# AllenNeuralDynamics/aind-exaspim-image-compression

Measured on AMD Instinct MI355X. Metric: denoised+encoded voxels/s on 1024^3 uint16, higher is better.
Workload: dtype f32

## Files before the change

aind-exaspim-image-compression_amd/csrc/bm_kernels.hip:

```cpp
#include "exabm4d_kernels.h"
#ifdef EXABM4D_BM_STAMPS
#define KERNEL_STAMPS
#endif
#include "kernel_stamps.h"
#include <type_traits>
#include <utility>

namespace exabm4d {

#ifdef EXABM4D_BM_STAMPS
__device__ unsigned long long g_bm_stamps[8];
__device__ unsigned long long g_bm_barrier_stamps[4][8];
#endif

struct __attribute__((packed, aligned(4))) float4u {
    float x, y, z, w;
};
template <class F, int... I>
__device__ __forceinline__ void static_for(F&& f, std::integer_sequence<int, I...>) {
    (f(std::integral_constant<int, I>{}), ...);
}

constexpr int TCZ = 8;
constexpr int NE = 6;
constexpr int NSTEP = SWIN * 2 * 4;
template <int TCY_, int TCX_>
struct TilePlan {
    static constexpr int TCY = TCY_, TCX = TCX_;
    static constexpr int TRY = TCY - 1, TRX = TCX - 1;
    static constexpr int PROWS = 4 * (TCY - 1) + 3 + NE;
    static_assert(TCY * TCX == 64, "one wave per cell layer");
};
template <int TCY_, int TCX_>
struct TileShape : TilePlan<TCY_, TCX_> {
    using Plan = TilePlan<TCY_, TCX_>;
    static constexpr int PCOLS = 4 * (TCX_ - 1) + 16;
    static constexpr int PSTR = TCX_ == 8 ? 56 : PCOLS;
    static constexpr int PCH = PSTR / 4;
    static constexpr int NDMA = (Plan::PROWS * PCH + 63) / 64;
    static constexpr int PLANE = (Plan::PROWS * PSTR + 3) / 4 * 4;
    static constexpr int PBUF = PLANE > 2144 ? PLANE : 2144;
    static_assert(PCOLS % 4 == 0 && PSTR % 4 == 0, "whole 16-byte chunks");
};

constexpr int CARRY_ROUND = (NE / 2) * SWIN * 64;
constexpr int CARRY_TILE = (NSTEP / 4) * 2 * CARRY_ROUND;
struct Carry {
    int on;
    int strip;
    uint32_t* buf;
    int* done;
    int* ticket;
    unsigned* status;
    int fault;
};
constexpr int CARRY_POLL_LIMIT = 1 << 23;
template <class T, class D>
__device__ __forceinline__ void carry_prefetch(const T* src, D* dst, int lane) {
    static_assert(2 * CARRY_ROUND == 16 * 256 + 128, "two rounds = 16.5 KB");
#pragma unroll
    for (int i = 0; i < 16; i++)
        __builtin_amdgcn_global_load_lds((const __attribute__((address_space(1))) void*)(src + 256 * i + 4 * lane),
                                         (__attribute__((address_space(3))) void*)(dst + 256 * i), 16, 0, 17);
    if (lane < 32)
        __builtin_amdgcn_global_load_lds((const __attribute__((address_space(1))) void*)(src + 4096 + 4 * lane),
                                         (__attribute__((address_space(3))) void*)(dst + 4096), 16, 0, 17);
}
__device__ __forceinline__ void carry_wait_for(const int* done, int tiles, int lane, const Carry& carry) {
    if (lane == 0) {
        int polls = carry.fault ? CARRY_POLL_LIMIT : 0;
        while (__hip_atomic_load(done, __ATOMIC_RELAXED, __HIP_MEMORY_SCOPE_SYSTEM) < tiles) {
            if (++polls > CARRY_POLL_LIMIT) {
                __hip_atomic_fetch_or(carry.status, 1u, __ATOMIC_RELAXED, __HIP_MEMORY_SCOPE_SYSTEM);
                break;
            }
            __builtin_amdgcn_s_sleep(32);
        }
        if (carry.fault) __hip_atomic_fetch_or(carry.status, 1u, __ATOMIC_RELAXED, __HIP_MEMORY_SCOPE_SYSTEM);
    }
}
__device__ __forceinline__ int launch_position(const Carry& carry, int quota) {
    if (!carry.on) return (int)blockIdx.x;
    __shared__ int s_pos;
    if (threadIdx.x == 0) {
        const int xcc = (int)(__builtin_amdgcn_s_getreg((4 - 1) << 11 | 0 << 6 | 20) & 7);
        int pos = -1;
        for (int k = 0; k < 8 && pos < 0; k++) {
            const int c = (xcc + k) & 7;
            const int j = __hip_atomic_fetch_add(carry.ticket + c, 1, __ATOMIC_RELAXED, __HIP_MEMORY_SCOPE_AGENT);
            if (j < quota) pos = 8 * j + c;
        }
        s_pos = pos;
    }
    __syncthreads();
    return s_pos;
}

struct TileId {
    int tz, col, cols;
    int bi, ty, tx;
};
__device__ __forceinline__ bool tile_id(TileId& t, int tiles_y, int tiles_x, int xcd_q, int nbatch,
                                        const Carry& carry) {
    const int per = tiles_y * tiles_x;
    t.cols = per * nbatch;
    if (xcd_q) {
        const int lp = launch_position(carry, (int)(gridDim.x >> 3));
        const int s = lp < 0 ? -1 : xcd_slab_sync(lp, t.cols, xcd_q);
        if (s < 0) return false;
        t.tz = s / t.cols;
        t.col = s - t.tz * t.cols;
    } else {
// ... 245 lines not shown
                            const uint32_t cbase =
                                1u + (uint32_t)(((dz + RAD) * SWIN + (dy + RAD)) * SWIN);
                            const bool self_row = (dz == 0) && (dy == 0);
#pragma unroll
                            for (int d = 0; d < SWIN; d++) {
                                const float* c0 = lo_w + (cz == 0 && e0 ? CARRY_ROUND : 0) + 64 * ((e - e0) * SWIN + d);
                                const float* c1 = up_w + 64 * ((e - e0) * SWIN + d);
                                float s0 = c0[0] + c0[TCX];
                                asm("" : "+v"(s0));
                                const float s1 = c1[0] + c1[TCX];
                                const float S = s0 + s1;
                                const uint32_t code = (d == RAD && self_row) ? 0u : cbase + d;
                                const bool valid = vzy && ((xmask >> d) & 1u);
                                list_admit(list, thr, keymax, __float_as_uint(S), code, valid);
                            }
                        }
                    }
                }
                __syncthreads();
                if (carries) {
#pragma unroll
                    for (int e = e0; e < e0 + NE / 2; e++)
#pragma unroll
                        for (int d = 0; d < SWIN; d++) {
                            const float right = __int_as_float(__builtin_amdgcn_update_dpp(
                                0, __float_as_int(acc[e][d]), 0x101 , 0xF, 0xF, true));
                            __hip_atomic_store(cslot + (e0 ? CARRY_ROUND : 0) + 64 * ((e - e0) * SWIN + d), acc[e][d] + right,
                                               __ATOMIC_RELAXED, __HIP_MEMORY_SCOPE_SYSTEM);
                        }
                }
            }
#pragma unroll
            for (int e = 0; e < NE; e++)
#pragma unroll
                for (int d = 0; d < SWIN; d++) acc[e][d] = 0.0f;
        }

        if (!xin && step + 1 < NSTEP) stage_edge(step + 1, nxt);
    }

    if (ref_ok) list_store(keys + ((size_t)((size_t)iz * g.gy + iy) * g.gx + ix) * MAXG, list);
    } while (false);

    if (carry.on) {
        asm volatile("s_waitcnt vmcnt(0)" ::: "memory");
        __syncthreads();
        if (threadIdx.x == 0) __hip_atomic_store(done_col, tz + 1, __ATOMIC_RELAXED, __HIP_MEMORY_SCOPE_SYSTEM);
    }
}

typedef short s16x2 __attribute__((ext_vector_type(2)));
typedef uint32_t u32x2 __attribute__((ext_vector_type(2)));
typedef uint32_t u32x4 __attribute__((ext_vector_type(4)));
template <int TCY_, int TCX_>
struct TileShape16 : TilePlan<TCY_, TCX_> {
    using Plan = TilePlan<TCY_, TCX_>;
    static constexpr int PCOLS = ((4 * TCX_ + 10 + 7) / 8) * 8;
    static constexpr int PSTR = TCX_ == 8 ? 56 : 80;
    static constexpr int PCH = PSTR / 8;
    static constexpr int NDMA = (Plan::PROWS * PCH + 63) / 64;
    static constexpr int PLANE_DW = NDMA * 256;
    static constexpr int XCH_DW = (NE / 2) * SWIN * 64;
    static constexpr int PBUF = PLANE_DW > XCH_DW ? PLANE_DW : XCH_DW;
    static_assert(PCOLS <= PSTR, "staged columns fit the row");
};

template <class TS>
__global__ __launch_bounds__(512) void bm_tile16_kernel(const uint16_t* __restrict__ vol_all, VolGeom g,
                                                        uint32_t keymax,
                                                        uint32_t* __restrict__ keys_all, int tiles_y,
                                                        int tiles_x, int xcd_q, int nbatch, Carry carry) {
    constexpr int TCX = TS::TCX, TRX = TS::TRX, TRY = TS::TRY, PROWS = TS::PROWS, PCOLS = TS::PCOLS,
                  PSTR = TS::PSTR, PCH = TS::PCH, NDMA = TS::NDMA, PBUF = TS::PBUF;
    __shared__ __align__(16) uint32_t pbuf_all[TCZ][2][PBUF];
    __shared__ __align__(16) uint32_t lower0[2 * CARRY_ROUND + 64];

    TileId id;
    if (!tile_id(id, tiles_y, tiles_x, xcd_q, nbatch, carry)) return;
    const int tz = id.tz, col = id.col, cols = id.cols, bi = id.bi, ty = id.ty, tx = id.tx;
    const uint16_t* __restrict__ vol = vol_all + (size_t)bi * (size_t)g.nvox;
    uint32_t* __restrict__ keys = keys_all + (size_t)bi * (size_t)g.nref * MAXG;
    const int tid = threadIdx.x;
    const int lane = tid & 63;
    const int cx = lane % TCX, cy = lane / TCX, cz = __builtin_amdgcn_readfirstlane(tid >> 6);
    const int ix = TRX * tx + cx, iy = TRY * ty + cy;
    const size_t sy = (size_t)g.nx, sz = (size_t)g.nx * (size_t)g.ny;
#ifdef EXABM4D_BM_STAMPS
    unsigned long long st[8] = {}, stb[4] = {};
    const unsigned long long tk0 = stamp();
#endif

    const int Ls = (carry.on ? TCZ : TCZ - 1) * tz;
    const uint32_t* carry_rd = carry.buf + ((size_t)((tz + 1) & 1) * cols + col) * CARRY_TILE;
    uint32_t* carry_wr = carry.buf + ((size_t)(tz & 1) * cols + col) * CARRY_TILE;
    int* done_col = carry.done + col;

    const int qy = min(STEP * iy, g.ny - STEP), qx = min(STEP * ix, g.nx - STEP);
    const int Y0 = STEP * TRY * ty, X0 = STEP * TRX * tx - RAD - 1;
    const int ry = STEP * iy, rx = STEP * ix;
    const bool ref_yx = cx < TRX && cy < TRY && iy < g.ay && ix < g.ax;

    uint32_t xmask = 0;
#pragma unroll
    for (int d = 0; d < SWIN; d++)
        xmask |= ((rx + d - RAD >= 0) && (rx + d - RAD <= g.nx - BLK)) ? (1u << d) : 0u;

    do {
    const int L = Ls + cz;
    const bool active = L <= g.az;
    const int iz = L - 1;
    const int qz = min(STEP * L, g.nz - STEP);
    const int Z0 = STEP * L;
    const bool lower_carried = carry.on && cz == 0 && tz > 0;
    const bool carries = carry.on && cz == TCZ - 1 && L + 1 <= g.az;
    const bool ref_ok = ref_yx && active && (cz > 0 || lower_carried);
    {
        STAMP(c0);
        if ((lower_carried || carries) && tz > 0) carry_wait_for(done_col, tz, lane, carry);
        STAMP(c1);
        STAMP_ADD(6, c0, c1);
    }
    const int rz = STEP * iz;

    uint32_t list[MAXG];
#pragma unroll
    for (int k = 0; k < MAXG; k++) list[k] = KEY_EMPTY;
    uint32_t thr = keymax;

    uint32_t doff[2][NDMA], coff[4];
    int yb[2];
    {
        int l = lane;
        asm volatile("" : "+v"(l));
#pragma unroll
        for (int ps = 0; ps < 2; ps++) {
            const int dylo = ps == 0 ? -RAD : 1;
            yb[ps] = min(max(Y0 + dylo, 0), g.ny - 1);
#pragma unroll
            for (int i = 0; i < NDMA; i++) {
                const unsigned p = 64u * i + (unsigned)l;
                const unsigned r0 = (p * (65536u / PCH + 1u)) >> 16;
                const unsigned r = min(r0, (unsigned)(PROWS - 1));
                const unsigned q = min(p - r0 * PCH, (unsigned)(PCOLS / 8 - 1));
                const int yy = min(max(Y0 + dylo + (int)r, 0), g.ny - 1);
                doff[ps][i] = 2u * ((unsigned)(yy - yb[ps]) * (unsigned)g.nx + 8u * q);
                asm volatile("" : "+v"(doff[ps][i]));
            }
        }
#pragma unroll
        for (int y = 0; y < 4; y++) {
            coff[y] = 2u * ((unsigned)(qy - Y0 + y) * (unsigned)g.nx + (unsigned)qx);
            asm volatile("" : "+v"(coff[y]));
        }
    }
    const char* const vol_b = reinterpret_cast<const char*>(vol);
    u32x2 An[4];
    auto load_cell_plane = [&](int step) {
        const char* cbase = vol_b + 2 * ((long long)(qz + (step & 3)) * (long long)sz + (long long)Y0 * (long long)sy);
#pragma unroll
        for (int y = 0; y < 4; y++) {
            uint32_t o = coff[y];
            asm volatile("" : "+v"(o));
            const uint32_t* ap = reinterpret_cast<const uint32_t*>(cbase + (size_t)o);
            An[y] = u32x2{ap[0], ap[1]};
        }
    };

    using lds_u32 = __attribute__((address_space(3))) uint32_t;
    auto pbuf = [&](int w, int b) { return (lds_u32*)&pbuf_all[w][b][0]; };
    auto issue_dma = [&](int step, lds_u32* dst) {
        const int z = step & 3, pass = (step >> 2) & 1, dz = (step >> 3) - RAD;
        const int pz = min(max(Z0 + z + dz, 0), g.nz - 1);
        const int yb0 = yb[0], yb1 = yb[1];
        const char* base = vol_b + 2 * ((long long)pz * (long long)sz +
                                        (long long)(pass ? yb1 : yb0) * (long long)sy + X0);
#pragma unroll
        for (int i = 0; i < NDMA; i++) {
            const uint32_t o0 = doff[0][i], o1 = doff[1][i];
            __builtin_amdgcn_global_load_lds(
                (const __attribute__((address_space(1))) void*)(base + (size_t)(pass ? o1 : o0)),
                (__attribute__((address_space(3))) void*)(dst + 256 * i), 16, 0, 0);
        }
    };

    if (!active) {
        for (int i = 0; i < (NSTEP / 4) * 4; i++) __syncthreads();
        break;
    }
    issue_dma(0, pbuf(cz, 0));
    load_cell_plane(0);
    asm volatile("" ::"v"(An[0]), "v"(An[1]), "v"(An[2]), "v"(An[3]));

    int acc[NE][SWIN];
#pragma unroll
    for (int e = 0; e < NE; e++)
#pragma unroll
        for (int d = 0; d < SWIN; d++) acc[e][d] = 0;

    auto step_body = [&](auto NEc, const int step) {
        constexpr int NEP = decltype(NEc)::value;
        const int z = step & 3;
        lds_u32* cur = pbuf(cz, step & 1);
        lds_u32* nxt = pbuf(cz, (step + 1) & 1);

        STAMP(t0);
        asm volatile("s_waitcnt vmcnt(0)" ::: "memory");
        STAMP(t1);
        (void)load_cell_plane;
        const u32x2 A[4] = {An[0], An[1], An[2], An[3]};
        STAMP(t2);
        if (step + 1 < NSTEP) issue_dma(step + 1, nxt);
        if (lower_carried && z == 2)
            carry_prefetch(carry_rd + (size_t)(step >> 2) * 2 * CARRY_ROUND, (lds_u32*)&lower0[0], lane);
        if (step + 1 < NSTEP) load_cell_plane(step + 1);
        asm volatile("" ::: "memory");
        STAMP(t3);

        {
            const lds_u32* wrow_l = cur + ((4 * cy) * PSTR + 4 * cx) / 2;
            const uint32_t wrow_lds = (uint32_t)(uintptr_t)wrow_l;
            auto read_row = [&](auto rc, u32x4& lo, u32x4& hi) {
                constexpr int r = decltype(rc)::value;
                constexpr int O = r * (PSTR / 4);
                static_assert(O + 3 < 256, "ds_read2_b64 offsets are 8 bits");
                const uint32_t row0 = wrow_lds;
                asm volatile("ds_read2_b64 %0, %2 offset0:%3 offset1:%4\n\t"
                             "ds_read2_b64 %1, %2 offset0:%5 offset1:%6"
                             : "=&v"(lo), "=&v"(hi)
                             : "v"(row0), "n"(O), "n"(O + 1), "n"(O + 2), "n"(O + 3));
            };
            auto await_row = [&](u32x4& lo, u32x4& hi) {
                asm volatile("s_waitcnt lgkmcnt(0)" : "+v"(lo), "+v"(hi));
            };
            u32x4 q0, q1;
            read_row(std::integral_constant<int, 0>{}, q0, q1);
            await_row(q0, q1);
            STAMP(t4);
            static_for([&](auto rc) {
                constexpr int rp = decltype(rc)::value;
                u32x4 n0, n1;
                if constexpr (rp + 1 < 3 + NEP) read_row(std::integral_constant<int, rp + 1>{}, n0, n1);
                asm volatile("" ::: "memory");
                const uint32_t W[8] = {q0.x, q0.y, q0.z, q0.w, q1.x, q1.y, q1.z, q1.w};
                uint32_t Wo[7];
#pragma unroll
                for (int i = 0; i < 7; i++) Wo[i] = __builtin_amdgcn_alignbit(W[i + 1], W[i], 16);
#pragma unroll
                for (int y = 0; y < 4; y++) {
                    const int e = rp - y;
                    if (e >= 0 && e < NEP) {
#pragma unroll
                        for (int xp = 0; xp < 2; xp++) {
                            const s16x2 a = __builtin_bit_cast(s16x2, xp ? A[y].y : A[y].x);
#pragma unroll
                            for (int d = 0; d < SWIN; d++) {
                                const int j = 1 + 2 * xp + d;
                                const uint32_t wp = (j & 1) ? Wo[(j - 1) / 2] : W[j / 2];
                                const s16x2 t = __builtin_elementwise_sub_sat(a, __builtin_bit_cast(s16x2, wp));
                                acc[e][d] = __builtin_amdgcn_sdot2(t, t, acc[e][d], true);
                            }
                        }
                    }
                }
                if constexpr (rp + 1 < 3 + NEP) {
                    await_row(n0, n1);
                    q0 = n0;
                    q1 = n1;
                }
            }, std::make_integer_sequence<int, 3 + NEP>{});
            asm volatile("" ::: "memory");
            STAMP(t5);
            STAMP_ADD(0, t0, t1);
            STAMP_ADD(1, t1, t2);
            STAMP_ADD(2, t3, t4);
            STAMP_ADD(3, t4, t5);
        }
    };
    auto pass_end = [&](auto NEc, const int step) {
        constexpr int NEP = decltype(NEc)::value;
        constexpr int NR0 = (NEP + 1) / 2;
        const int dz = (step >> 3) - RAD;
        const int dylo = NEP == NE ? -RAD : 1;
        lds_u32* cur = pbuf(cz, step & 1);
        {
            const bool vz = (rz + dz >= 0) && (rz + dz <= g.nz - BLK);
            lds_u32* mine = cur + lane;
            const lds_u32* up_w = cur + lane;
            const lds_u32* lo_w = (cz > 0 ? pbuf(max(cz - 1, 0), step & 1) : (lds_u32*)&lower0[0]) + lane;
            uint32_t* cslot = carry_wr + (size_t)((step >> 2) * 2) * CARRY_ROUND + lane;
            auto pair_sum = [&](int e, int d) {
                const uint32_t c = min((uint32_t)acc[e][d], 1u << 27);
                const uint32_t right = (uint32_t)__builtin_amdgcn_update_dpp(
                    0, (int)c, 0x101 , 0xF, 0xF, true);
                return c + right;
            };
#pragma unroll
            for (int e0 = 0; e0 < NEP; e0 += NR0) {
#pragma unroll
                for (int e = e0; e < (e0 + NR0 < NEP ? e0 + NR0 : NEP); e++)
#pragma unroll
                    for (int d = 0; d < SWIN; d++) mine[64 * ((e - e0) * SWIN + d)] = pair_sum(e, d);
                STAMP(b0);
                __syncthreads();
                STAMP(b1);
                if (ref_ok) {
#pragma unroll
                    for (int e = e0; e < (e0 + NR0 < NEP ? e0 + NR0 : NEP); e++) {
                        uint32_t Sv[1][SWIN];
#pragma unroll
                        for (int d = 0; d < SWIN; d++) {
                            const lds_u32* c0 = lo_w + (cz == 0 && e0 ? CARRY_ROUND : 0) + 64 * ((e - e0) * SWIN + d);
                            const lds_u32* c1 = up_w + 64 * ((e - e0) * SWIN + d);
                            Sv[0][d] = (c0[0] + c0[TCX]) + (c1[0] + c1[TCX]);
                        }
                        asm volatile("" ::: "memory");
                        const int dy = dylo + e;
                        {
                            const bool vzy = vz && (ry + dy >= 0) && (ry + dy <= g.ny - BLK);
                            const uint32_t cbase =
                                1u + (uint32_t)(((dz + RAD) * SWIN + (dy + RAD)) * SWIN);
                            const bool self_row = (dz == 0) && (dy == 0);
#pragma unroll
                            for (int d = 0; d < SWIN; d++) {
                                const uint32_t S = Sv[0][d];
                                const uint32_t code = (d == RAD && self_row) ? 0u : cbase + d;
                                const bool valid = vzy && ((xmask >> d) & 1u);
                                list_admit(list, thr, keymax, __float_as_uint((float)S), code, valid);
                            }
                        }
                    }
                }
                STAMP(b2);
                __syncthreads();
                STAMP(b3);
                STAMP_ADD(4, b0, b1);
                STAMP_ADD(5, b1, b2);
                STAMP_ADD(4, b2, b3);
#ifdef EXABM4D_BM_STAMPS
                stb[e0 ? 2 : 0] += b1 - b0;
                stb[e0 ? 3 : 1] += b3 - b2;
#endif
                if (carries) {
                    uint32_t* cw = cslot + (size_t)(e0 ? CARRY_ROUND : 0);
#pragma unroll
                    for (int e = e0; e < (e0 + NR0 < NEP ? e0 + NR0 : NEP); e++)
#pragma unroll
                        for (int d = 0; d < SWIN; d++)
                            __hip_atomic_store(cw + 64 * ((e - e0) * SWIN + d), pair_sum(e, d), __ATOMIC_RELAXED,
                                               __HIP_MEMORY_SCOPE_SYSTEM);
                }
            }
#pragma unroll
            for (int e = 0; e < NE; e++)
#pragma unroll
                for (int d = 0; d < SWIN; d++) acc[e][d] = 0;
        }
    };
    static_assert(NSTEP == 8 * SWIN, "two passes of four planes per dz");
#pragma unroll 1
    for (int step0 = 0; step0 < NSTEP; step0 += 8) {
#pragma unroll 1
        for (int step = step0; step < step0 + 4; step++) step_body(std::integral_constant<int, NE>{}, step);
        pass_end(std::integral_constant<int, NE>{}, step0 + 3);
#pragma unroll 1
        for (int step = step0 + 4; step < step0 + 8; step++) step_body(std::integral_constant<int, NE - 1>{}, step);
        pass_end(std::integral_constant<int, NE - 1>{}, step0 + 7);
    }

    if (ref_ok) list_store(keys + ((size_t)((size_t)iz * g.gy + iy) * g.gx + ix) * MAXG, list);
    } while (false);

    if (carry.on) {
        STAMP(c0);
        asm volatile("s_waitcnt vmcnt(0)" ::: "memory");
        __syncthreads();
        STAMP(c1);
        STAMP_ADD(6, c0, c1);
        if (threadIdx.x == 0) __hip_atomic_store(done_col, tz + 1, __ATOMIC_RELAXED, __HIP_MEMORY_SCOPE_SYSTEM);
    }
#ifdef EXABM4D_BM_STAMPS
    st[7] = stamp() - tk0;
    if (lane == 0)
        for (int i = 0; i < 8; i++) atomicAdd(&g_bm_stamps[i], st[i]);
    if (lane == 0)
        for (int i = 0; i < 4; i++) atomicAdd(&g_bm_barrier_stamps[i][tid >> 6], stb[i]);
#endif
}

#ifdef EXABM4D_BM_STAMPS
extern "C" void exabm4d_debug_bm_stamps(unsigned long long* out, int reset) {
    unsigned long long z[8] = {};
    (void)hipDeviceSynchronize();
    (void)hipMemcpyFromSymbol(out, HIP_SYMBOL(g_bm_stamps), sizeof(z));
    if (reset) (void)hipMemcpyToSymbol(HIP_SYMBOL(g_bm_stamps), z, sizeof(z));
}
extern "C" void exabm4d_debug_bm_barrier_stamps(unsigned long long* out, int reset) {
    unsigned long long z[4][8] = {};
    (void)hipDeviceSynchronize();
    (void)hipMemcpyFromSymbol(out, HIP_SYMBOL(g_bm_barrier_stamps), sizeof(z));
    if (reset) (void)hipMemcpyToSymbol(HIP_SYMBOL(g_bm_barrier_stamps), z, sizeof(z));
}
#endif

__global__ __launch_bounds__(64) void bm_generic_kernel(const float* __restrict__ vol_all,
                                                        VolGeom g, uint32_t keymax,
                                                        uint32_t* __restrict__ keys_all,
                                                        int only_unaligned) {
    __shared__ float rb[BVOX];
    const float* __restrict__ vol = vol_all + (size_t)blockIdx.y * (size_t)g.nvox;
    uint32_t* __restrict__ keys = keys_all + (size_t)blockIdx.y * (size_t)g.nref * MAXG;

    const long long r = blockIdx.x;
    const int ix = (int)(r % g.gx), iy = (int)((r / g.gx) % g.gy),
              iz = (int)(r / ((long long)g.gx * g.gy));
    if (only_unaligned && iz < g.az && iy < g.ay && ix < g.ax) return;
    const int rz = grid_pos(iz, g.az, g.nz), ry = grid_pos(iy, g.ay, g.ny),
              rx = grid_pos(ix, g.ax, g.nx);
    const size_t sy = (size_t)g.nx, sz = (size_t)g.nx * (size_t)g.ny;
    const int lane = threadIdx.x;

    for (int i = lane; i < BVOX; i += 64) {
        const int bx = i & 7, by = (i >> 3) & 7, bz = i >> 6;
        rb[i] = vol[(size_t)(rz + bz) * sz + (size_t)(ry + by) * sy + (rx + bx)];
    }
    __syncthreads();

    uint32_t list[MAXG];
#pragma unroll
    for (int k = 0; k < MAXG; k++) list[k] = KEY_EMPTY;

    for (int c = lane; c < NCAND; c += 64) {
        const int dx = c % SWIN - RAD, dy = (c / SWIN) % SWIN - RAD, dz = c / (SWIN * SWIN) - RAD;
        const int pz = rz + dz, py = ry + dy, px = rx + dx;
        const bool valid = pz >= 0 && pz <= g.nz - BLK && py >= 0 && py <= g.ny - BLK && px >= 0 &&
                           px <= g.nx - BLK;
        uint32_t key = KEY_EMPTY;
        if (valid) {
            const float* __restrict__ b = vol + (size_t)pz * sz + (size_t)py * sy + px;
            float cell[8];
#pragma unroll 1
            for (int kc = 0; kc < 8; kc++) {
                const int kz = kc >> 2, ky = (kc >> 1) & 1, kx = kc & 1;
                float acc = 0.0f;
#pragma unroll 1
                for (int z = 0; z < 4; z++)
#pragma unroll
                    for (int y = 0; y < 4; y++) {
                        const int bz = 4 * kz + z, by = 4 * ky + y;
                        const float* bp = b + (size_t)bz * sz + (size_t)by * sy + 4 * kx;
                        const float* ap = rb + (bz * 8 + by) * 8 + 4 * kx;
#pragma unroll
                        for (int x = 0; x < 4; x++) {
                            const float t = ap[x] - bp[x];
                            acc = fmaf(t, t, acc);
                        }
                    }
                cell[kc] = acc;
            }
            const float lo = (cell[0] + cell[1]) + (cell[2] + cell[3]);
            const float hi = (cell[4] + cell[5]) + (cell[6] + cell[7]);
            const float S = lo + hi;
            key = (__float_as_uint(S) & KEY_DMASK) | disp_code(dz, dy, dx);
            if (key >= keymax) key = KEY_EMPTY;
        }
        list_insert(list, key);
    }

    uint32_t* out = keys + (size_t)r * MAXG;
    for (int k = 0; k < MAXG; k++) {
        uint32_t m = list[0];
#pragma unroll
        for (int off = 32; off >= 1; off >>= 1) m = min(m, (uint32_t)__shfl_xor((int)m, off));
        if (list[0] == m && m != KEY_EMPTY) {
#pragma unroll
            for (int i = 0; i < MAXG - 1; i++) list[i] = list[i + 1];
            list[MAXG - 1] = KEY_EMPTY;
        }
        if (lane == 0) out[k] = (k == 0 && m == KEY_EMPTY) ? 0u : m;
    }
}


using Cube = TilePlan<8, 8>;
using Flat = TilePlan<4, 16>;
static bool flat_tiles(const VolGeom& g) {
    auto tiles = [&](int try_, int trx) {
        return (long long)((g.ay + try_ - 1) / try_) * ((g.ax + trx - 1) / trx);
    };
    return tiles(Flat::TRY, Flat::TRX) < tiles(Cube::TRY, Cube::TRX);
}
BmPlan bm_plan(const VolGeom& g, int batch, const BmOpts& opt) {
    BmPlan p = {};
    if (g.az <= 0 || g.ay <= 0 || g.ax <= 0) return p;
    p.flat = flat_tiles(g) ? 1 : 0;
    const int try_ = p.flat ? Flat::TRY : Cube::TRY, trx = p.flat ? Flat::TRX : Cube::TRX;
    p.ty = (g.ay + try_ - 1) / try_;
    p.tx = (g.ax + trx - 1) / trx;
    const long long cols = (long long)p.ty * p.tx * batch;
    const int tz7 = (g.az + TCZ - 2) / (TCZ - 1), tz8 = g.az / TCZ + 1;
    const bool slab = opt.xcd_mode != 0 && cols >= 512;
    const bool worth = tz8 >= 2 && tz8 < tz7 && slab;
    const size_t need = 2 * (size_t)cols * CARRY_TILE * sizeof(uint32_t) + ((size_t)cols + 64) * sizeof(int);
    p.carry = (opt.carry != 0 && (worth || (opt.carry == 2 && tz8 >= 2)) && need <= ((size_t)16 << 30)) ? 1 : 0;
    p.carry_bytes = p.carry ? need : 0;
    p.tz = p.carry ? tz8 : tz7;
    p.xq = (p.carry || (slab && p.tz >= 2)) ? (int)((cols + 7) / 8) : 0;
    p.strip = (opt.xcd_mode >= 2 && p.xq) ? opt.xcd_mode : 0;
    p.fault = opt.carry_fault;
    return p;
}

hipError_t launch_blockmatch(const float* vol, const VolGeom& g, int batch, uint32_t keymax,
                             uint32_t* keys, hipStream_t stream, int force_generic, int guarded,
                             const uint16_t* vol16, const BmPlan& p, void* carry_mem, unsigned* status) {
    if (p.carry && (!carry_mem || !status)) return hipErrorInvalidValue;
    if (!force_generic && g.az > 0 && g.ay > 0 && g.ax > 0) {
        Carry carry;
        carry.strip = p.strip;
        carry.on = p.carry;
        carry.buf = static_cast<uint32_t*>(carry_mem);
        const size_t cols = (size_t)p.ty * p.tx * (size_t)batch;
        carry.done = p.carry ? reinterpret_cast<int*>(carry.buf + 2 * cols * CARRY_TILE) : nullptr;
        carry.ticket = p.carry ? carry.done + cols : nullptr;
        carry.status = status;
        carry.fault = p.fault;
        if (p.carry) {
            hipError_t e = hipMemsetAsync(carry.done, 0, (cols + 8) * sizeof(int), stream);
            if (e != hipSuccess) return e;
        }
        if (vol16 &&
            ((unsigned long long)Cube::PROWS * (unsigned long long)g.nx + 80ull) * 2ull >= (1ull << 32))
            return hipErrorInvalidValue;
        const dim3 grid((unsigned)(p.xq ? 8 * p.xq * p.tz : p.tz * p.ty * p.tx), (unsigned)(p.xq ? 1 : batch));
        auto launch = [&](auto plan) {
            using Shape16 = TileShape16<decltype(plan)::TCY, decltype(plan)::TCX>;
            using Shape = TileShape<decltype(plan)::TCY, decltype(plan)::TCX>;
            if (vol16)
                hipLaunchKernelGGL(bm_tile16_kernel<Shape16>, grid, dim3(512), 0, stream, vol16, g, keymax, keys,
                                   p.ty, p.tx, p.xq, batch, carry);
            else
                hipLaunchKernelGGL(bm_tile_kernel<Shape>, grid, dim3(512), 0, stream, vol, g, keymax, keys, p.ty,
                                   p.tx, guarded, p.xq, batch, carry);
        };
        if (p.flat)
            launch(Flat{});
        else
            launch(Cube{});
        hipError_t e = hipGetLastError();
        if (e != hipSuccess) return e;
    }
    const bool unaligned = g.gz != g.az || g.gy != g.ay || g.gx != g.ax;
    if (force_generic || unaligned) {
        dim3 grid((unsigned)g.nref, (unsigned)batch);
        hipLaunchKernelGGL(bm_generic_kernel, grid, dim3(64), 0, stream, vol, g, keymax, keys,
                           force_generic ? 0 : 1);
        return hipGetLastError();
    }
    return hipSuccess;
}

}
```

aind-exaspim-image-compression_amd/csrc/exabm4d_api.hip:

```cpp
#include <initializer_list>
#include <new>

#include "exabm4d_api.h"

using namespace exabm4d;

static thread_local std::string g_err;

namespace exabm4d {

int fail(exabm4d_ctx* ctx, int code, const std::string& msg) {
    g_err = msg;
    if (ctx) ctx->err = msg;
    return code;
}

static double bessel_i0(double x) {
    double sum = 1.0, term = 1.0, q = x * x / 4.0;
    for (int k = 1; k < 200; k++) {
        term *= q / ((double)k * (double)k);
        sum += term;
        if (term < 1e-18 * sum) break;
    }
    return sum;
// ... 215 lines not shown
    HIP_TRY(ctx, hipStreamCreateWithFlags(&ctx->stream, hipStreamNonBlocking));
    ctx->own_stream = true;
    return check_async_status(ctx);
}

int exabm4d_sync(exabm4d_ctx* ctx) {
    if (!ctx) return fail(nullptr, EXABM4D_ERR_INVALID, "ctx is NULL");
    HIP_TRY(ctx, hipStreamSynchronize(ctx->stream));
    return check_async_status(ctx);
}

int exabm4d_default_params(exabm4d_params* p) {
    if (!p) return fail(nullptr, EXABM4D_ERR_INVALID, "params is NULL");
    p->size = sizeof(exabm4d_params);
    p->block = 8;
    p->step = 4;
    p->search = 11;
    p->max_group = 16;
    p->lambda_ht = 2.7f;
    p->c_match_ht = 3.0f;
    p->c_match_wie = 0.6f;
    p->kaiser_beta = 2.0f;
    return EXABM4D_OK;
}

int exabm4d_set_option(exabm4d_ctx* ctx, const char* name, int value) {
    if (!ctx || !name) return fail(ctx, EXABM4D_ERR_INVALID, "NULL argument");
    if (std::strcmp(name, "force_generic_bm") == 0) {
        ctx->force_generic_bm = value ? 1 : 0;
        return EXABM4D_OK;
    }
    if (std::strcmp(name, "bm_guarded_copy") == 0) {
        ctx->bm_guarded_copy = value ? 1 : 0;
        return EXABM4D_OK;
    }
    if (std::strcmp(name, "codec_version") == 0) {
        if (value != 1 && value != 2) return fail(ctx, EXABM4D_ERR_INVALID, "codec_version must be 1 or 2");
        ctx->codec_version = value;
        return EXABM4D_OK;
    }
    if (std::strcmp(name, "bm_int") == 0) {
        ctx->bm_int = value ? 1 : 0;
        return EXABM4D_OK;
    }
    if (std::strcmp(name, "stage_pairvol") == 0) {
        ctx->stage.pairvol = value ? 1 : 0;
        return EXABM4D_OK;
    }
    if (std::strcmp(name, "bm_carry") == 0) {
        if (value < 0 || value > 2) return fail(ctx, EXABM4D_ERR_INVALID, "bm_carry must be 0, 1 or 2");
        ctx->bm.carry = value;
        return EXABM4D_OK;
    }
    if (std::strcmp(name, "host_pipeline") == 0) {
        ctx->host_pipeline = value ? 1 : 0;
        return EXABM4D_OK;
    }
    if (std::strcmp(name, "zero_overlap") == 0) {
        ctx->zero_overlap = value ? 1 : 0;
        return EXABM4D_OK;
    }
    if (std::strcmp(name, "bm_carry_fault") == 0) {
        ctx->bm.carry_fault = value ? 1 : 0;
        return EXABM4D_OK;
    }
    if (std::strcmp(name, "bm_xcd_mode") == 0) {
        ctx->bm.xcd_mode = value < 0 ? 0 : (value > 16 ? 16 : value);
        return EXABM4D_OK;
    }
    if (std::strcmp(name, "stage_strip") == 0) {
        ctx->stage.strip = value > 0 ? value : 0;
        return EXABM4D_OK;
    }
    if (std::strcmp(name, "stage_chunks") == 0) {
        ctx->stage.chunks = value > 0 ? value : 0;
        return EXABM4D_OK;
    }
    if (std::strcmp(name, "chunk_budget_mb") == 0) {
        if (value < 1) return fail(ctx, EXABM4D_ERR_INVALID, "chunk_budget_mb must be >= 1");
        ctx->chunk_budget_mb = value;
        return EXABM4D_OK;
    }
    if (std::strcmp(name, "profile") == 0) {
        if (value && !ctx->ev[0])
            for (int i = 0; i < 2 * EXABM4D_PHASE_COUNT; i++) HIP_TRY(ctx, hipEventCreate(&ctx->ev[i]));
        ctx->profile = value ? 1 : 0;
        return EXABM4D_OK;
    }
    return fail(ctx, EXABM4D_ERR_INVALID, std::string("unknown option: ") + name);
}

int exabm4d_malloc(exabm4d_ctx* ctx, size_t bytes, void** dptr) {
    if (!ctx || !dptr) return fail(ctx, EXABM4D_ERR_INVALID, "NULL argument");
    *dptr = nullptr;
    HIP_TRY(ctx, hipSetDevice(ctx->device));
    hipError_t e = hipMalloc(dptr, bytes ? bytes : 1);
    if (e != hipSuccess) return fail(ctx, EXABM4D_ERR_NOMEM, std::string("hipMalloc: ") + hipGetErrorString(e));
    return EXABM4D_OK;
}
int exabm4d_free(exabm4d_ctx* ctx, void* dptr) {
    if (!ctx) return fail(nullptr, EXABM4D_ERR_INVALID, "ctx is NULL");
    if (dptr) {
        HIP_TRY(ctx, hipStreamSynchronize(ctx->stream));
        HIP_TRY(ctx, hipFree(dptr));
    }
    return EXABM4D_OK;
// ... 9 lines not shown
    if (int rc = fetch(ctx, dst, src, bytes)) return rc;
    return check_async_status(ctx);
}
int exabm4d_memset(exabm4d_ctx* ctx, void* dst, int value, size_t bytes) {
    if (!ctx || (!dst && bytes)) return fail(ctx, EXABM4D_ERR_INVALID, "NULL argument");
    HIP_TRY(ctx, hipMemsetAsync(dst, value, bytes, ctx->stream));
    return EXABM4D_OK;
}
int exabm4d_event_create(exabm4d_ctx* ctx, void** ev) {
    if (!ctx || !ev) return fail(ctx, EXABM4D_ERR_INVALID, "NULL argument");
    hipEvent_t e;
    HIP_TRY(ctx, hipEventCreate(&e));
    *ev = (void*)e;
    return EXABM4D_OK;
}
int exabm4d_event_destroy(exabm4d_ctx* ctx, void* ev) {
    if (!ctx) return fail(nullptr, EXABM4D_ERR_INVALID, "ctx is NULL");
    if (ev) HIP_TRY(ctx, hipEventDestroy((hipEvent_t)ev));
    return EXABM4D_OK;
}
int exabm4d_event_record(exabm4d_ctx* ctx, void* ev) {
    if (!ctx || !ev) return fail(ctx, EXABM4D_ERR_INVALID, "NULL argument");
    HIP_TRY(ctx, hipEventRecord((hipEvent_t)ev, ctx->stream));
    return EXABM4D_OK;
}
int exabm4d_event_elapsed_ms(exabm4d_ctx* ctx, void* a, void* b, float* ms) {
    if (!ctx || !a || !b || !ms) return fail(ctx, EXABM4D_ERR_INVALID, "NULL argument");
    HIP_TRY(ctx, hipEventSynchronize((hipEvent_t)b));
    HIP_TRY(ctx, hipEventElapsedTime(ms, (hipEvent_t)a, (hipEvent_t)b));
    return EXABM4D_OK;
}

int exabm4d_grid_count(int n) { return grid_count(n); }
int exabm4d_grid_positions(int n, int32_t* pos) {
    if (!pos) return fail(nullptr, EXABM4D_ERR_INVALID, "pos is NULL");
    const int c = grid_count(n), a = aligned_count(n);
    for (int i = 0; i < c; i++) pos[i] = grid_pos(i, a, n);
    return EXABM4D_OK;
}
int exabm4d_tables(const exabm4d_params* p, float* dct64, float* win512) {
    int rc = check_params(nullptr, p);
    if (rc) return rc;
    if (!dct64 || !win512) return fail(nullptr, EXABM4D_ERR_INVALID, "NULL argument");
    make_tables((double)p->kaiser_beta, dct64, win512);
    return EXABM4D_OK;
}
int exabm4d_blockmatch_plan(const exabm4d_ctx* ctx, int nz, int ny, int nx, int batch, int32_t plan[6],
                            uint64_t* carry_bytes) {
    if (!plan || !carry_bytes) return EXABM4D_ERR_INVALID;
    VolGeom g;
    const int rc = make_geom(nullptr, nz, ny, nx, batch, g);
    if (rc) return rc;
    const BmPlan p = bm_plan(g, batch, ctx ? ctx->bm : BmOpts());
    plan[0] = p.tz; plan[1] = p.ty; plan[2] = p.tx; plan[3] = p.xq; plan[4] = p.carry; plan[5] = p.flat;
    *carry_bytes = (uint64_t)p.carry_bytes;
    return EXABM4D_OK;
}

int exabm4d_host_register(exabm4d_ctx* ctx, void* ptr, size_t bytes) {
    if (!ctx || !ptr || !bytes) return fail(ctx, EXABM4D_ERR_INVALID, "NULL argument or empty range");
    HIP_TRY(ctx, hipSetDevice(ctx->device));
    HIP_TRY(ctx, hipHostRegister(ptr, bytes, hipHostRegisterDefault));
    return EXABM4D_OK;
}
int exabm4d_host_unregister(exabm4d_ctx* ctx, void* ptr) {
    if (!ctx || !ptr) return fail(ctx, EXABM4D_ERR_INVALID, "NULL argument");
    HIP_TRY(ctx, hipSetDevice(ctx->device));
    HIP_TRY(ctx, hipStreamSynchronize(ctx->stream));
    HIP_TRY(ctx, hipHostUnregister(ptr));
    return EXABM4D_OK;
}

int exabm4d_profile_read(exabm4d_ctx* ctx, float* ms, int max_phases) {
    if (!ctx || !ms) return fail(ctx, EXABM4D_ERR_INVALID, "NULL argument");
    if (!ctx->ev[0]) return fail(ctx, EXABM4D_ERR_INVALID, "profiling was never enabled");
    HIP_TRY(ctx, hipStreamSynchronize(ctx->stream));
    int n = max_phases < EXABM4D_PHASE_COUNT ? max_phases : EXABM4D_PHASE_COUNT;
    for (int i = 0; i < n; i++) {
        ms[i] = 0.0f;
        if (ctx->ev_used[i]) HIP_TRY(ctx, hipEventElapsedTime(&ms[i], ctx->ev[2 * i], ctx->ev[2 * i + 1]));
    }
    return n;
}

}
```

aind-exaspim-image-compression_amd/csrc/exabm4d_kernels.h:

```cpp
#pragma once
#include "exabm4d_common.h"

namespace exabm4d {

struct TfDev {
    int kind;
    int wrapped;
    float woff;
    float maxc;
    float off, scale, norm;
    float gain, c38g2, rn2, two_over_gain, cinvg2;
    float mn, fden, clip, range;
};

struct PgDev {
    int inverse;
    float gain, off, c38g2, rn2, two_over_gain;
    float cg2;
    float d0, s2, k1, k2, k3;
};
hipError_t launch_pg_forward_u16(const PgDev& t, const uint16_t* in, float* out, size_t n, hipStream_t s);
hipError_t launch_pg_inverse_u16(const PgDev& t, const float* in, uint16_t* out, size_t n, hipStream_t s);

hipError_t launch_normalize(const float* num, const float* den, float* out, size_t n, float lo,
// ... 89 lines not shown
    unsigned tiles[3];
};
hipError_t foreground_prepare();
bool foreground_box_plan(const uint16_t* win, const BoxGeom& g, int radius, const uint16_t* out16, const uint8_t* out8,
                         FgPlan& p);
hipError_t launch_foreground_box_u16(const uint16_t* win, const BoxGeom& g, const FgPlan& p, uint32_t cut, int radius,
                                     uint32_t value, uint16_t* out16, uint8_t* out8, unsigned long long* counts,
                                     hipStream_t s);
constexpr int CC_TZ = 8, CC_TY = 8, CC_TX = 64;
struct CcGeom {
    int w0[3], wd[3], r0[3], rd[3], b0[3], bd[3], c0[3], cd[3];
    unsigned tiles[3];
    long long voxels, box_voxels;
};
bool components_geometry(const BoxGeom& b, const int* count0, const int* countd, long long grow, CcGeom& g);
size_t components_scratch_bytes(long long voxels);
hipError_t launch_components(const void* win, bool win_u8, const CcGeom& g, uint32_t cut, uint32_t min_voxels,
                             int connectivity, uint32_t* parent, uint32_t* labels, uint32_t* sizes, uint16_t* out16,
                             uint8_t* out8, unsigned long long* counts, hipStream_t s);
struct SegGeom {
    int n[3], w0[3], wd[3], b0[3], bd[3];
    long long voxels, brick_voxels;
};
long long segment_halo_records(const SegGeom& g);
long long segment_face_records(const SegGeom& g);
hipError_t launch_segment_collect(const uint32_t* labels, const SegGeom& g, uint32_t* own, unsigned long long* halo,
                                  unsigned long long halo_cap, unsigned long long* face, unsigned long long face_cap,
                                  unsigned long long* size, unsigned long long size_cap, unsigned long long* counts,
                                  hipStream_t s);
hipError_t launch_segment_relabel(const uint32_t* labels, const SegGeom& g, const unsigned long long* keys,
                                  const unsigned long long* vals, unsigned long long n_keys, int typesize, void* final,
                                  void* out, hipStream_t s);
hipError_t launch_nonzero_u8(const uint16_t* src, uint8_t* dst, size_t n, hipStream_t s);
constexpr int DS_MODE = 0, DS_MEAN = 1, DS_MAX = 2;
constexpr int DS_CROP = 0, DS_PARTIAL = 1;
struct DsPlan {
    int f[3];
    int ox, pieces;
    int vec_in, vec_out;
    unsigned block[2], grid[3];
};
void downsample_box_plan(const uint16_t* win, const BoxGeom& g, const int* factors, const uint16_t* out, DsPlan& p);
hipError_t launch_downsample_box_u16(const uint16_t* win, const BoxGeom& g, const DsPlan& p, int method, uint16_t* out,
                                     hipStream_t s);
constexpr int LABEL_ZEROS_COUNT = 0, LABEL_ZEROS_IGNORE = 1;
void label_downsample_box_plan(const void* win, int typesize, const BoxGeom& g, const int* factors, const void* out,
                               DsPlan& p);
hipError_t launch_downsample_box_labels(const void* win, int typesize, const BoxGeom& g, const DsPlan& p, int zeros,
                                        void* out, hipStream_t s);
struct BmOpts {
    int xcd_mode = 2;
    int carry = 1;
    int carry_fault = 0;
};
struct BmPlan {
    int tz, ty, tx;
    int xq;
    int carry;
    int flat;
    int strip, fault;
    size_t carry_bytes;
};
BmPlan bm_plan(const VolGeom& g, int batch, const BmOpts& opt);
hipError_t launch_blockmatch(const float* vol, const VolGeom& g, int batch, uint32_t keymax,
                             uint32_t* keys, hipStream_t stream, int force_generic, int guarded,
                             const uint16_t* vol16, const BmPlan& plan, void* carry_mem, unsigned* status);
struct StageOpts {
    int pairvol = 1;
    int strip = 3;
    int chunks = 0;
};
hipError_t launch_stage(const float* noisy, const float* basic, const uint32_t* keys,
                        const VolGeom& g, int batch, const float* dct64, const float* win_dev,
                        float thr, float sigma2, const double* qscale, long long* num,
                        unsigned long long* cw, hipStream_t stream, const StageOpts& opt,
                        float* pair = nullptr, int pair_ready = 0);
hipError_t launch_qscale(const float* vol, size_t nvox, int batch, int fixed_exp, unsigned* maxbits,
                         double* qscale, hipStream_t s, unsigned* status = nullptr);
hipError_t launch_den_from_corners(const unsigned long long* cw, float* tmp, float* den, int nz, int ny, int nx,
                                   int batch, const float* win1d, hipStream_t s);
hipError_t launch_den_xy_from_corners(const unsigned long long* cw, float* tmp, int nz, int ny, int nx, int batch,
                                      const float* win1d, hipStream_t s);
struct NormOut {
    float* f32; bool clip; float lo, hi;
    uint16_t* u16; float offset; const PgDev* pg;
    static NormOut to_f32(float* out) { return {out, false, 0.0f, 0.0f, nullptr, 0.0f, nullptr}; }
    static NormOut to_f32_abi_clip(float* out, float clip_lo, float clip_hi) {
        return {out, clip_lo <= clip_hi, clip_lo, clip_hi, nullptr, 0.0f, nullptr};
    }
    static NormOut to_u16(uint16_t* out, float offset) { return {nullptr, false, 0.0f, 0.0f, out, offset, nullptr}; }
    static NormOut to_u16_pg(uint16_t* out, const PgDev* pg) { return {nullptr, false, 0.0f, 0.0f, out, 0.0f, pg}; }
};
struct NormSums {
    const long long* num; const double* qscale; const float* txy;
    int nz, ny, nx, batch;
    const float* win1d;
};
struct NormSide { const float* pair_src; float* pair_out; uint16_t* round16; float round_offset; };
struct NormWrote { hipError_t err; bool pair, round16; };
NormWrote launch_normalize_zconv(const NormSums& in, const NormOut& out, hipStream_t s, const NormSide* side = nullptr);
size_t groupnorm_workspace_bytes(int batch, size_t spatial, int C, int G);
template <typename T>
hipError_t launch_groupnorm_lrelu_ndhwc(const T* x, T* y, int batch, size_t spatial, int C, int G,
                                        const float* gamma, const float* beta, float eps, float slope,
                                        void* workspace, hipStream_t s, const float* cbias = nullptr,
                                        float* stats = nullptr);
template <typename T>
hipError_t launch_maxpool2_ndhwc(const T* x, T* y, int batch, int D, int H, int W, int C, hipStream_t s);
template <typename T>
// ... 211 lines not shown
```

Before: 2.039 billion.

## Add 12-layer block-matching tiles for uint16 path with LDS-budgeted exchange rounds

Templates the uint16 block-matching kernel on the number of z cell layers per workgroup and adds a 12-layer (768-thread) variant. The exchange buffer rows per round are sized from the per-CU LDS budget, so a pass may need more barrier rounds. The planner picks 12 layers automatically when carry is on and a cost heuristic says fewer z tiles will pay off. The aim is to cut redundant plane loads and carry handoffs across z tiles, at the cost of more barriers per pass and lower occupancy from the larger workgroup.

```diff
diff --git a/aind-exaspim-image-compression_amd/csrc/bm_kernels.hip b/aind-exaspim-image-compression_amd/csrc/bm_kernels.hip
--- a/aind-exaspim-image-compression_amd/csrc/bm_kernels.hip
+++ b/aind-exaspim-image-compression_amd/csrc/bm_kernels.hip
@@ -10,7 +10,8 @@
 
 #ifdef EXABM4D_BM_STAMPS
 __device__ unsigned long long g_bm_stamps[8];
-__device__ unsigned long long g_bm_barrier_stamps[4][8];
+constexpr int BM_STAMP_BARRIERS = 6, BM_STAMP_WAVES = 12;
+__device__ unsigned long long g_bm_barrier_stamps[BM_STAMP_BARRIERS][BM_STAMP_WAVES];
 #endif
 
 struct __attribute__((packed, aligned(4))) float4u {
@@ -57,7 +58,7 @@
 constexpr int CARRY_POLL_LIMIT = 1 << 23;
 template <class T, class D>
 __device__ __forceinline__ void carry_prefetch(const T* src, D* dst, int lane) {
-    static_assert(2 * CARRY_ROUND == 16 * 256 + 128, "two rounds = 16.5 KB");
+    static_assert(2 * CARRY_ROUND == 16 * 256 + 128, "a slot = 16.5 KB");
 #pragma unroll
     for (int i = 0; i < 16; i++)
         __builtin_amdgcn_global_load_lds((const __attribute__((address_space(1))) void*)(src + 256 * i + 4 * lane),
@@ -409,28 +410,41 @@
 typedef short s16x2 __attribute__((ext_vector_type(2)));
 typedef uint32_t u32x2 __attribute__((ext_vector_type(2)));
 typedef uint32_t u32x4 __attribute__((ext_vector_type(4)));
-template <int TCY_, int TCX_>
+constexpr int LDS_CU_BYTES = 160 * 1024;
+constexpr int LOWER0_DW = 2 * CARRY_ROUND + 64;
+template <int TCY_, int TCX_, int LAYERS_ = TCZ>
 struct TileShape16 : TilePlan<TCY_, TCX_> {
     using Plan = TilePlan<TCY_, TCX_>;
+    static constexpr int LAYERS = LAYERS_;
     static constexpr int PCOLS = ((4 * TCX_ + 10 + 7) / 8) * 8;
     static constexpr int PSTR = TCX_ == 8 ? 56 : 80;
     static constexpr int PCH = PSTR / 8;
     static constexpr int NDMA = (Plan::PROWS * PCH + 63) / 64;
     static constexpr int PLANE_DW = NDMA * 256;
-    static constexpr int XCH_DW = (NE / 2) * SWIN * 64;
+    static constexpr int BUF_BUDGET_DW = ((LDS_CU_BYTES - 16) / 4 - LOWER0_DW) / (2 * LAYERS);
+    static constexpr int XROWS_FIT = BUF_BUDGET_DW / (SWIN * 64);
+    static constexpr int XROWS = XROWS_FIT < NE / 2 ? XROWS_FIT : NE / 2;
+    static constexpr int XCH_DW = XROWS * SWIN * 64;
     static constexpr int PBUF = PLANE_DW > XCH_DW ? PLANE_DW : XCH_DW;
+    static constexpr int LDS_BYTES = (LAYERS * 2 * PBUF + LOWER0_DW) * 4 + 16;
+    static constexpr int rounds(int rows) { return (rows + XROWS - 1) / XROWS; }
+    static constexpr int TILE_BARRIERS = SWIN * 2 * (rounds(NE) + rounds(NE - 1));
     static_assert(PCOLS <= PSTR, "staged columns fit the row");
+    static_assert(XROWS >= 1 && PBUF >= PLANE_DW && PBUF >= XCH_DW, "a buffer holds a plane and an exchange round");
+    static_assert(LDS_BYTES <= LDS_CU_BYTES, "one workgroup's LDS fits the CU");
+    static_assert(64 * LAYERS <= 1024, "one wave per cell layer");
 };
 
 template <class TS>
-__global__ __launch_bounds__(512) void bm_tile16_kernel(const uint16_t* __restrict__ vol_all, VolGeom g,
+__global__ __launch_bounds__(64 * TS::LAYERS) void bm_tile16_kernel(const uint16_t* __restrict__ vol_all, VolGeom g,
                                                         uint32_t keymax,
                                                         uint32_t* __restrict__ keys_all, int tiles_y,
                                                         int tiles_x, int xcd_q, int nbatch, Carry carry) {
     constexpr int TCX = TS::TCX, TRX = TS::TRX, TRY = TS::TRY, PROWS = TS::PROWS, PCOLS = TS::PCOLS,
-                  PSTR = TS::PSTR, PCH = TS::PCH, NDMA = TS::NDMA, PBUF = TS::PBUF;
-    __shared__ __align__(16) uint32_t pbuf_all[TCZ][2][PBUF];
-    __shared__ __align__(16) uint32_t lower0[2 * CARRY_ROUND + 64];
+                  PSTR = TS::PSTR, PCH = TS::PCH, NDMA = TS::NDMA, PBUF = TS::PBUF, LAYERS = TS::LAYERS,
+                  XROWS = TS::XROWS;
+    __shared__ __align__(16) uint32_t pbuf_all[LAYERS][2][PBUF];
+    __shared__ __align__(16) uint32_t lower0[LOWER0_DW];
 
     TileId id;
     if (!tile_id(id, tiles_y, tiles_x, xcd_q, nbatch, carry)) return;
@@ -443,11 +457,11 @@
     const int ix = TRX * tx + cx, iy = TRY * ty + cy;
     const size_t sy = (size_t)g.nx, sz = (size_t)g.nx * (size_t)g.ny;
 #ifdef EXABM4D_BM_STAMPS
-    unsigned long long st[8] = {}, stb[4] = {};
+    unsigned long long st[8] = {}, stb[BM_STAMP_BARRIERS] = {};
     const unsigned long long tk0 = stamp();
 #endif
 
-    const int Ls = (carry.on ? TCZ : TCZ - 1) * tz;
+    const int Ls = (carry.on ? LAYERS : LAYERS - 1) * tz;
     const uint32_t* carry_rd = carry.buf + ((size_t)((tz + 1) & 1) * cols + col) * CARRY_TILE;
     uint32_t* carry_wr = carry.buf + ((size_t)(tz & 1) * cols + col) * CARRY_TILE;
     int* done_col = carry.done + col;
@@ -469,7 +483,7 @@
     const int qz = min(STEP * L, g.nz - STEP);
     const int Z0 = STEP * L;
     const bool lower_carried = carry.on && cz == 0 && tz > 0;
-    const bool carries = carry.on && cz == TCZ - 1 && L + 1 <= g.az;
+    const bool carries = carry.on && cz == LAYERS - 1 && L + 1 <= g.az;
     const bool ref_ok = ref_yx && active && (cz > 0 || lower_carried);
     {
         STAMP(c0);
@@ -541,7 +555,7 @@
     };
 
     if (!active) {
-        for (int i = 0; i < (NSTEP / 4) * 4; i++) __syncthreads();
+        for (int i = 0; i < TS::TILE_BARRIERS; i++) __syncthreads();
         break;
     }
     issue_dma(0, pbuf(cz, 0));
@@ -635,7 +649,11 @@
     };
     auto pass_end = [&](auto NEc, const int step) {
         constexpr int NEP = decltype(NEc)::value;
-        constexpr int NR0 = (NEP + 1) / 2;
+        constexpr int NR0 = XROWS, NROUND = TS::rounds(NEP);
+        static_assert((NROUND - 1) * NR0 < NEP && NROUND * NR0 >= NEP, "the rounds cover the pass's rows, none is empty");
+#ifdef EXABM4D_BM_STAMPS
+        static_assert(2 * NROUND <= BM_STAMP_BARRIERS, "a stamp slot per barrier");
+#endif
         const int dz = (step >> 3) - RAD;
         const int dylo = NEP == NE ? -RAD : 1;
         lds_u32* cur = pbuf(cz, step & 1);
@@ -666,7 +684,7 @@
                         uint32_t Sv[1][SWIN];
 #pragma unroll
                         for (int d = 0; d < SWIN; d++) {
-                            const lds_u32* c0 = lo_w + (cz == 0 && e0 ? CARRY_ROUND : 0) + 64 * ((e - e0) * SWIN + d);
+                            const lds_u32* c0 = lo_w + (cz == 0 && e0 ? e0 * SWIN * 64 : 0) + 64 * ((e - e0) * SWIN + d);
                             const lds_u32* c1 = up_w + 64 * ((e - e0) * SWIN + d);
                             Sv[0][d] = (c0[0] + c0[TCX]) + (c1[0] + c1[TCX]);
                         }
@@ -694,11 +712,11 @@
                 STAMP_ADD(5, b1, b2);
                 STAMP_ADD(4, b2, b3);
 #ifdef EXABM4D_BM_STAMPS
-                stb[e0 ? 2 : 0] += b1 - b0;
-                stb[e0 ? 3 : 1] += b3 - b2;
+                stb[2 * (e0 / NR0)] += b1 - b0;
+                stb[2 * (e0 / NR0) + 1] += b3 - b2;
 #endif
                 if (carries) {
-                    uint32_t* cw = cslot + (size_t)(e0 ? CARRY_ROUND : 0);
+                    uint32_t* cw = cslot + (size_t)(e0 ? e0 * SWIN * 64 : 0);
 #pragma unroll
                     for (int e = e0; e < (e0 + NR0 < NEP ? e0 + NR0 : NEP); e++)
 #pragma unroll
@@ -714,6 +732,8 @@
         }
     };
     static_assert(NSTEP == 8 * SWIN, "two passes of four planes per dz");
+    static_assert(TS::TILE_BARRIERS == (NSTEP / 8) * 2 * (TS::rounds(NE) + TS::rounds(NE - 1)),
+                  "idle and working waves pass the same number of barriers");
 #pragma unroll 1
     for (int step0 = 0; step0 < NSTEP; step0 += 8) {
 #pragma unroll 1
@@ -740,7 +760,7 @@
     if (lane == 0)
         for (int i = 0; i < 8; i++) atomicAdd(&g_bm_stamps[i], st[i]);
     if (lane == 0)
-        for (int i = 0; i < 4; i++) atomicAdd(&g_bm_barrier_stamps[i][tid >> 6], stb[i]);
+        for (int i = 0; i < BM_STAMP_BARRIERS; i++) atomicAdd(&g_bm_barrier_stamps[i][tid >> 6], stb[i]);
 #endif
 }
 
@@ -752,7 +772,7 @@
     if (reset) (void)hipMemcpyToSymbol(HIP_SYMBOL(g_bm_stamps), z, sizeof(z));
 }
 extern "C" void exabm4d_debug_bm_barrier_stamps(unsigned long long* out, int reset) {
-    unsigned long long z[4][8] = {};
+    unsigned long long z[BM_STAMP_BARRIERS][BM_STAMP_WAVES] = {};
     (void)hipDeviceSynchronize();
     (void)hipMemcpyFromSymbol(out, HIP_SYMBOL(g_bm_barrier_stamps), sizeof(z));
     if (reset) (void)hipMemcpyToSymbol(HIP_SYMBOL(g_bm_barrier_stamps), z, sizeof(z));
@@ -840,6 +860,7 @@
 
 using Cube = TilePlan<8, 8>;
 using Flat = TilePlan<4, 16>;
+constexpr double BM_LAYER_COST_12_OVER_8 = 0.92;
 static bool flat_tiles(const VolGeom& g) {
     auto tiles = [&](int try_, int trx) {
         return (long long)((g.ay + try_ - 1) / try_) * ((g.ax + trx - 1) / trx);
@@ -854,14 +875,25 @@
     p.ty = (g.ay + try_ - 1) / try_;
     p.tx = (g.ax + trx - 1) / trx;
     const long long cols = (long long)p.ty * p.tx * batch;
-    const int tz7 = (g.az + TCZ - 2) / (TCZ - 1), tz8 = g.az / TCZ + 1;
+    auto tz7_of = [&](int l) { return (g.az + l - 2) / (l - 1); };
+    auto tz8_of = [&](int l) { return g.az / l + 1; };
     const bool slab = opt.xcd_mode != 0 && cols >= 512;
-    const bool worth = tz8 >= 2 && tz8 < tz7 && slab;
     const size_t need = 2 * (size_t)cols * CARRY_TILE * sizeof(uint32_t) + ((size_t)cols + 64) * sizeof(int);
-    p.carry = (opt.carry != 0 && (worth || (opt.carry == 2 && tz8 >= 2)) && need <= ((size_t)16 << 30)) ? 1 : 0;
+    const bool fits = need <= ((size_t)16 << 30);
+    auto worth_of = [&](int l) { return tz8_of(l) >= 2 && tz8_of(l) < tz7_of(l) && slab; };
+    int layers = TCZ;
+    if (opt.layers == 12 && !p.flat) layers = 12;
+    if (opt.layers == 0 && !p.flat && opt.carry != 0 && fits && worth_of(TCZ) && worth_of(12) &&
+        tz8_of(12) * 12 * BM_LAYER_COST_12_OVER_8 <= tz8_of(TCZ) * TCZ)
+        layers = 12;
+    p.layers = layers;
+    const int tz7 = tz7_of(layers), tz8 = tz8_of(layers);
+    const bool worth = worth_of(layers);
+    p.carry = (opt.carry != 0 && (worth || (opt.carry == 2 && tz8 >= 2)) && fits) ? 1 : 0;
     p.carry_bytes = p.carry ? need : 0;
     p.tz = p.carry ? tz8 : tz7;
-    p.xq = (p.carry || (slab && p.tz >= 2)) ? (int)((cols + 7) / 8) : 0;
+    p.tz_f32 = p.carry ? tz8_of(TCZ) : tz7_of(TCZ);
+    p.xq = (p.carry || (slab && (p.tz >= 2 || p.tz_f32 >= 2))) ? (int)((cols + 7) / 8) : 0;
     p.strip = (opt.xcd_mode >= 2 && p.xq) ? opt.xcd_mode : 0;
     p.fault = opt.carry_fault;
     return p;
@@ -888,17 +920,24 @@
         if (vol16 &&
             ((unsigned long long)Cube::PROWS * (unsigned long long)g.nx + 80ull) * 2ull >= (1ull << 32))
             return hipErrorInvalidValue;
-        const dim3 grid((unsigned)(p.xq ? 8 * p.xq * p.tz : p.tz * p.ty * p.tx), (unsigned)(p.xq ? 1 : batch));
+        if (p.layers != TCZ && (p.layers != 12 || p.flat)) return hipErrorInvalidValue;
+        const int tz = vol16 ? p.tz : p.tz_f32;
+        const dim3 grid((unsigned)(p.xq ? 8 * p.xq * tz : tz * p.ty * p.tx), (unsigned)(p.xq ? 1 : batch));
         auto launch = [&](auto plan) {
             using Shape16 = TileShape16<decltype(plan)::TCY, decltype(plan)::TCX>;
             using Shape = TileShape<decltype(plan)::TCY, decltype(plan)::TCX>;
             if (vol16)
-                hipLaunchKernelGGL(bm_tile16_kernel<Shape16>, grid, dim3(512), 0, stream, vol16, g, keymax, keys,
-                                   p.ty, p.tx, p.xq, batch, carry);
+                hipLaunchKernelGGL(bm_tile16_kernel<Shape16>, grid, dim3(64 * Shape16::LAYERS), 0, stream, vol16, g,
+                                   keymax, keys, p.ty, p.tx, p.xq, batch, carry);
             else
                 hipLaunchKernelGGL(bm_tile_kernel<Shape>, grid, dim3(512), 0, stream, vol, g, keymax, keys, p.ty,
                                    p.tx, guarded, p.xq, batch, carry);
         };
+        if (vol16 && p.layers == 12) {
+            using Shape12 = TileShape16<Cube::TCY, Cube::TCX, 12>;
+            hipLaunchKernelGGL(bm_tile16_kernel<Shape12>, grid, dim3(64 * Shape12::LAYERS), 0, stream, vol16, g, keymax,
+                               keys, p.ty, p.tx, p.xq, batch, carry);
+        } else
         if (p.flat)
             launch(Flat{});
         else
diff --git a/aind-exaspim-image-compression_amd/csrc/exabm4d_api.hip b/aind-exaspim-image-compression_amd/csrc/exabm4d_api.hip
--- a/aind-exaspim-image-compression_amd/csrc/exabm4d_api.hip
+++ b/aind-exaspim-image-compression_amd/csrc/exabm4d_api.hip
@@ -291,6 +291,11 @@
         ctx->bm.carry = value;
         return EXABM4D_OK;
     }
+    if (std::strcmp(name, "bm_layers") == 0) {
+        if (value != 0 && value != 8 && value != 12) return fail(ctx, EXABM4D_ERR_INVALID, "bm_layers must be 0, 8 or 12");
+        ctx->bm.layers = value;
+        return EXABM4D_OK;
+    }
     if (std::strcmp(name, "host_pipeline") == 0) {
         ctx->host_pipeline = value ? 1 : 0;
         return EXABM4D_OK;
@@ -406,7 +411,7 @@
     const int rc = make_geom(nullptr, nz, ny, nx, batch, g);
     if (rc) return rc;
     const BmPlan p = bm_plan(g, batch, ctx ? ctx->bm : BmOpts());
-    plan[0] = p.tz; plan[1] = p.ty; plan[2] = p.tx; plan[3] = p.xq; plan[4] = p.carry; plan[5] = p.flat;
+    plan[0] = p.tz_f32; plan[1] = p.ty; plan[2] = p.tx; plan[3] = p.xq; plan[4] = p.carry; plan[5] = p.flat;
     *carry_bytes = (uint64_t)p.carry_bytes;
     return EXABM4D_OK;
 }
diff --git a/aind-exaspim-image-compression_amd/csrc/exabm4d_kernels.h b/aind-exaspim-image-compression_amd/csrc/exabm4d_kernels.h
--- a/aind-exaspim-image-compression_amd/csrc/exabm4d_kernels.h
+++ b/aind-exaspim-image-compression_amd/csrc/exabm4d_kernels.h
@@ -165,9 +165,12 @@
     int xcd_mode = 2;
     int carry = 1;
     int carry_fault = 0;
+    int layers = 0;
 };
 struct BmPlan {
     int tz, ty, tx;
+    int layers;
+    int tz_f32;
     int xq;
     int carry;
     int flat;
```

Result: faster. 2.081 billion, median of 6 (+2.1%).
